# RizaXudayi/VarNet

Measured on AMD Instinct MI355X. Metric: training-points/sec (test-funcs x quad-pts), 2D+t AD-PDE, higher is better.
Workload: dtype f32

## Files before the change

varnet_amd/csrc/vn_fused16.hip:

```cpp
#include "vn_internal.h"
#include "vn_fused16_common.h"

namespace {
using namespace vn16;

constexpr int TSW = 132;
__host__ __device__ constexpr int t_rows(int KS) { return KS == 13 ? 52 : KS <= 8 ? 33 : 64; }
template <int KS>
__device__ __forceinline__ int trow(int pos) {
  if (KS == 13) return pos < 50 ? pos : pos == 52 ? 51 : 50;
  if (KS <= 8) return pos < 32 ? pos : 32;
  return pos;
}
__host__ __device__ constexpr bool fullpos(int KS) { return KS == 16 || KS == 8; }
__host__ __device__ constexpr int vones(int KS) {
  if (fullpos(KS)) return 4 * KS - 1;
  for (int p = 0; p < 64; ++p)
    if (vks(p) >= KS) return p;
  return -1;
}
static_assert(vfeat(63) == 63 && vfeat(31) == 31 && vpos(7, 3) == 31, "position 4*KS-1 is feature 4*KS-1");
#ifndef VN_MERGED_ROUNDS
#define VN_MERGED_ROUNDS 1
#endif
__host__ __device__ constexpr bool merged_rounds(int L, int KS) { return VN_MERGED_ROUNDS && KS <= 8 && L >= 2; }
__host__ __device__ constexpr bool bf_sweeps(int L, int KS) { return KS == 13 && L >= 2 && L <= 5; }

template <int L, int KS>
struct Lay {
  static constexpr int HP = 4 * KS;
  static constexpr bool BF = bf_sweeps(L, KS);
  static constexpr int HPWS = BF ? IMG / 4 : al4(HP * WS);
  static constexpr int W1_OFF = 0;
  static constexpr int WH_OFF = al4(8 * WS);
  static constexpr int BI_OFF = WH_OFF + (L - 1) * HPWS;
  static constexpr int WO_OFF = BI_OFF + L * 64;
  static constexpr int MISC_OFF = WO_OFF + al4(4 * KS);
  static constexpr int T_OFF = MISC_OFF + 256;
  static constexpr int G1_SZ = (4 * KS0 + 1) * HP;
  static constexpr int GH_SZ = (HP + 1) * HP;
  static constexpr int GO_OFF = G1_SZ + (L - 1) * GH_SZ;
  static constexpr int G_SZ = al4(GO_OFF + HP + 1);
  static constexpr bool MERGE = merged_rounds(L, KS);
  static constexpr int T_IMG = (MERGE ? 2 : 1) * 2 * t_rows(KS) * TSW;
  static constexpr int T_H13 = (KS == 13) ? 27 * (NW * 64 + 4) : 0;
  static constexpr int T_MAX = T_IMG > T_H13 ? T_IMG : T_H13;
  static constexpr int T_SZ_SHARED = al4(T_MAX > G_SZ ? T_MAX : G_SZ);
  static constexpr bool G_LOW = (T_OFF + T_SZ_SHARED > 160 * 256) && G_SZ <= MISC_OFF;
  static constexpr int T_SZ = G_LOW ? al4(T_MAX) : T_SZ_SHARED;
  static constexpr int G_OFF = G_LOW ? 0 : T_OFF;
  static constexpr int SLOT_SZ = NW * 2 * 4 * 64;
  static constexpr bool SLOT_IN_T = G_LOW || (T_SZ - al4(G_SZ) >= SLOT_SZ);
  static constexpr int SLOT_OFF = G_LOW ? T_OFF : (SLOT_IN_T ? T_OFF + al4(G_SZ) : 0);
  static_assert(SLOT_IN_T || SLOT_SZ <= MISC_OFF, "thin-layer slots fit neither behind the gradient image nor over the weight images");
  static constexpr int ST_OFF = T_OFF + T_SZ;
  static constexpr int ST_LAYER = NW * 2 * 64 * 4;
  static constexpr int ST_FIT = (160 * 256 - ST_OFF) / ST_LAYER;
  static constexpr int NST = (BF || (KS != 13 && KS != 16) || L < 3) ? 0 : (ST_FIT < L - 1 ? ST_FIT : L - 1);
  static constexpr int TOTAL = ST_OFF + NST * ST_LAYER;
  static constexpr int NSTG = (!BF || L < 3) ? 0 : 1;
  static constexpr int NSTK = BF ? NSTG : NST;
  static_assert(!BF || TOTAL <= 160 * 256, "bf16-piece images must fit the LDS");
};


struct LaneC {
  int g, c;
  int offF;
  int offB0;
  int twr;
};

template <int KSA, int KSB>
struct WG {
  static constexpr int ONES = vones(KSA);
  static constexpr int MTA0 = (mtiles(KSA) > (ONES >> 4) + 1) ? mtiles(KSA) : (ONES >> 4) + 1;
  static constexpr int MTA = MTA0 == 3 ? 4 : MTA0;
  static constexpr int NTB0 = mtiles(KSB);
  static constexpr int NTB = NTB0 == 3 ? 4 : NTB0;
  static constexpr int NT = MTA * NTB;
  static constexpr int TPW = (NT >= NW) ? NT / NW : 1;
  static constexpr int NS = (NT >= NW) ? 1 : NW / NT;
  static constexpr int PTS = TILE / NS;
  static constexpr int PG = PTS / 4;
  static constexpr int ones_m = ONES >> 4;
  static constexpr int ones_i = ONES & 3;
  static constexpr int ones_g = (ONES >> 2) & 3;
  static_assert(NT == 1 || NT == 2 || NT == 4 || NT == 8 || NT == 16, "tile count must divide the waves");
  static_assert(NT < NW || NTB % TPW == 0, "a wave's tiles must share a row tile");
};



template <int KS>
__device__ __forceinline__ void t_write(float* T, const LaneC& lc, int ks, float v) {
  if (KS == 13 && ks == 12) {
    if (lc.g < 2) T[lc.twr + (48 - lc.g) * TSW] = v;
  } else {
    T[lc.twr + vpos(ks, 0) * TSW] = v;
  }
}

template <int KSA, int KSB, bool RAWA, bool TANH, bool MERGE, int NACC, class AV, class BV>
__device__ __forceinline__ void wgrad_layer(const AV& av, const AV& azd, const BV& bv, const BV& bt, float* TA,
                                            float* TB, const LaneC& lc, int wave, f32x4 (&acc)[NACC], bool ones_row) {
  using W = WG<KSA, KSB>;
  static_assert(NACC == W::TPW, "accumulator count");
  const int t0 = (W::NT >= NW) ? wave * W::TPW : wave % W::NT;
  const int sidx = (W::NT >= NW) ? 0 : wave / W::NT;
  const int m = t0 / W::NTB, n0 = t0 % W::NTB;
  const int goff = (W::PG == 32) ? 64 * (lc.g & 1) + 32 * (lc.g >> 1) : lc.g * W::PG;
  const int rdA = trow<KSA>(16 * m + lc.c) * TSW + sidx * W::PTS + goff;
  int rdBt[W::TPW];
#pragma unroll
  for (int t = 0; t < W::TPW; ++t) rdBt[t] = trow<KSB>(16 * (n0 + t) + lc.c) * TSW + sidx * W::PTS + goff;
  constexpr int T2 = MERGE ? 2 * t_rows(KSB) * TSW : 0;
  auto contract = [&](const float* TAh, const float* TBh) {
    f32x4 a4 = *reinterpret_cast<const f32x4a*>(&TAh[rdA]);
    f32x4 b4[W::TPW];
#pragma unroll
    for (int t = 0; t < W::TPW; ++t) b4[t] = *reinterpret_cast<const f32x4a*>(&TBh[rdBt[t]]);
#pragma unroll
    for (int j = 0; j < W::PG / 4; ++j) {
      f32x4 an = a4, bn[W::TPW];
#pragma unroll
      for (int t = 0; t < W::TPW; ++t) bn[t] = b4[t];
      if (j + 1 < W::PG / 4) {
        an = *reinterpret_cast<const f32x4a*>(&TAh[rdA + 4 * (j + 1)]);
#pragma unroll
        for (int t = 0; t < W::TPW; ++t)
          bn[t] = *reinterpret_cast<const f32x4a*>(&TBh[rdBt[t] + 4 * (j + 1)]);
      }
      __builtin_amdgcn_sched_barrier(0);
#pragma unroll
      for (int e = 0; e < 4; ++e)
#pragma unroll
        for (int t = 0; t < W::TPW; ++t) acc[t] = mfma16(a4[e], b4[t][e], acc[t]);
      __builtin_amdgcn_sched_barrier(0);
      a4 = an;
#pragma unroll
      for (int t = 0; t < W::TPW; ++t) b4[t] = bn[t];
    }
  };
#pragma unroll
// ... 372 lines not shown
  float* WH = lds + LY::WH_OFF;
  float* BI = lds + LY::BI_OFF;
  float* WO = lds + LY::WO_OFF;
  float* sInt = lds + LY::MISC_OFF;
  float* TA = lds + LY::T_OFF;
  float* TB = TA + t_rows(KS) * TSW;
  const unsigned t_base_bytes = (unsigned)((LY::T_OFF + wave * 64) * 4);
  float* Gacc = lds + LY::G_OFF;

  const int q = A.integ_num;
  const int pq_l = (wave * CW + (lane & 15)) % q;
  const int tf_l = (wave * CW + (lane & 15)) / q;
  const float tab_dnt = A.time_dependent ? A.fedNt[pq_l] : 0.f;
  const float tab_w = A.feW ? A.feW[pq_l] : 1.f;
  const float tab_N = A.feN[pq_l];
  const float bo = A.theta[net.boff[L + 1]];
  {
    const int d_in = net.d_in, H1 = net.H[1];
    constexpr int NSRC = (LY::HP * LY::HP + NTHREADS - 1) / NTHREADS;
    static_assert(8 * 64 <= NTHREADS, "layer 1: one parameter per thread");
    float v1 = 0.f, vh[L > 1 ? L - 1 : 1][NSRC];
    if (tid < d_in * H1) v1 = A.theta[net.woff[1] + tid];
#pragma unroll
    for (int l = 2; l <= (LY::BF ? 1 : L); ++l) {
      const int n = net.H[l - 1] * net.H[l];
      const float* src = A.theta + net.woff[l];
#pragma unroll
      for (int it = 0; it < NSRC; ++it) {
        const int j = tid + it * NTHREADS;
        vh[l - 2][it] = j < n ? src[j] : 0.f;
      }
    }
    static_assert(L * 64 <= NTHREADS && 4 * KS <= NTHREADS, "one bias / output weight per thread");
    float vb = 0.f, vo = 0.f;
    if (tid < L * 64) {
      const int l = tid / 64 + 1, idx = tid % 64;
      const int mt = idx >> 4, g = (idx >> 2) & 3, r = idx & 3;
      const int ks = 4 * mt + r, f = 4 * ks + g;
      vb = (ks < KS && f < net.H[l]) ? A.theta[net.boff[l] + f] : 0.f;
    }
    if (tid < 4 * KS) vo = (tid < net.H[L]) ? A.theta[net.woff[L + 1] + tid] : 0.f;
    static_assert(LY::BI_OFF % 4 == 0 && LY::T_OFF % 4 == 0 && LY::T_SZ % 4 == 0, "16-byte zero fill");
    const f32x4 z4 = {0.f, 0.f, 0.f, 0.f};
    for (int i = tid; i < (LY::BF ? LY::WH_OFF : LY::BI_OFF) / 4; i += NTHREADS) reinterpret_cast<f32x4a*>(lds)[i] = z4;
    for (int i = tid; i < LY::T_SZ / 4; i += NTHREADS) reinterpret_cast<f32x4a*>(lds + LY::T_OFF)[i] = z4;
    __syncthreads();
    if (tid < d_in * H1) {
      const int k = tid / H1, f = tid - k * H1;
      W1[k * WS + vpos(f >> 2, f & 3)] = v1;
    }
    if constexpr (LY::BF) stage_split_hidden<L, true>(net, A.theta, reinterpret_cast<char*>(WH), tid);
#pragma unroll
    for (int l = 2; l <= (LY::BF ? 1 : L); ++l) {
      float* Wl = WH + (l - 2) * LY::HPWS;
      const int Hout = net.H[l], n = net.H[l - 1] * Hout;
      const int dq = NTHREADS / Hout, dr = NTHREADS - dq * Hout;
      int k = tid / Hout, f = tid - k * Hout;
#pragma unroll
      for (int it = 0; it < NSRC; ++it) {
        if (tid + it * NTHREADS < n) Wl[k * WS + vpos(f >> 2, f & 3)] = vh[l - 2][it];
        f += dr; k += dq;
        if (f >= Hout) { f -= Hout; ++k; }
      }
    }
    if (tid < L * 64) BI[tid] = vb;
    if (tid < 4 * KS) WO[tid] = vo;
  }
  __syncthreads();

  LaneC lc;
  lc.g = lane >> 4;
  lc.c = lane & 15;
  lc.offF = lc.g * WS + lc.c;
  static_assert(16 * GE::MTM <= LY::HP, "backward fragment rows stay inside the weight image");
  static_assert(vfeat(16 + 5) == 16 + vfeat(5), "row tile m holds features fin(c) + 16m");
  lc.offB0 = vfeat(lc.c) * WS + 4 * lc.g;
  lc.twr = 4 * lc.g * TSW + wave * CW + lc.c;

  using W1G = WG<KS0, KS>;
  using WHG = WG<KS, KS>;
  constexpr bool HID13 = (KS == 13);
  constexpr int NHACC = HID13 ? 2 : WHG::TPW;
  constexpr int ST_L = LY::ST_LAYER / 4;
  f32x4a* stash = (LY::BF ? reinterpret_cast<f32x4a*>(A.stash) + (long)blockIdx.x * LY::NSTG * ST_L
                          : reinterpret_cast<f32x4a*>(lds + LY::ST_OFF)) + wave * 2 * 64 + lane;
  constexpr int WIN = 2 * IMG;
  const int rowb = split_row_base(lc.g, lc.c), trb = split_tr_base(lc.g, lc.c);
  auto win_base = [&](int lane_base, int l) {
    const char* wh = reinterpret_cast<const char*>(WH);
    if (l - 2 < 2) return wh + lane_base + (l - 2) * IMG;
    int b = lane_base + WIN;
    asm volatile("" : "+v"(b));
    return wh + b + (l - 4) * IMG;
  };
  f32x4 wacc1[W1G::TPW], wacch[L > 1 ? L - 1 : 1][NHACC];
  float woacc = 0.f, boacc = 0.f;
#pragma unroll
  for (int t = 0; t < W1G::TPW; ++t) wacc1[t] = f32x4{0.f, 0.f, 0.f, 0.f};
#pragma unroll
  for (int l = 0; l < (L > 1 ? L - 1 : 1); ++l)
#pragma unroll
    for (int t = 0; t < NHACC; ++t) {
      wacch[l][t] = f32x4{0.f, 0.f, 0.f, 0.f};
      if (l < LY::NSTK) stash[l * ST_L + t * 64] = wacch[l][t];
    }

  const bool thin_in = net.d_in <= 3;
  bool ones_h[L > 1 ? L - 1 : 1];
#pragma unroll
  for (int l = 2; l <= L; ++l) ones_h[l - 2] = !fullpos(KS) || net.H[l - 1] < 4 * KS;
  float bsum_h[L > 1 ? L - 1 : 1];
#pragma unroll
  for (int l = 0; l < (L > 1 ? L - 1 : 1); ++l) bsum_h[l] = 0.f;
  const int TT = TILE / q;
  const int TPTS = TT * q;
  const bool qtree = (TILE % q) == 0;
  const long ntiles_i = A.mode ? (A.nT + TILE - 1) / TILE : (A.n_k + TT - 1) / TT;
  const long ntiles = ntiles_i + (A.mode == 1 ? 0 : (A.nB + TILE - 1) / TILE);
  float loss_var = 0.f, loss_bc = 0.f, loss_ic = 0.f;
  const long nI = A.nB - A.bDof;
  const float cb = A.bDof > 0 ? 2.f * A.w0 * A.biDimVal / (float)A.bDof : 0.f;
  const float ci = nI > 0 ? 2.f * A.w1 * A.biDimVal / (float)nI : 0.f;
  enum : unsigned {
    FL_MODE1 = 1u << 0, FL_MODE2 = 1u << 1, FL_DIR = 1u << 2, FL_TD = 1u << 3, FL_DNTROW = 1u << 4, FL_SRC = 1u << 5,
    FL_NROW = 1u << 6, FL_QTREE = 1u << 7, FL_DETJV = 1u << 8, FL_LOSSVEC = 1u << 9, FL_SEEDU = 1u << 10, FL_SEEDUD = 1u << 11,
    FL_OUTU = 1u << 12, FL_OUTUD = 1u << 13, FL_THIN_IN = 1u << 14
  };
  const unsigned flags = (A.mode == 1 ? FL_MODE1 : 0u) | (A.mode == 2 ? FL_MODE2 : 0u) | (A.dir >= 0 ? FL_DIR : 0u) |
                         (A.time_dependent ? FL_TD : 0u) | (A.dNtrow ? FL_DNTROW : 0u) | (A.src ? FL_SRC : 0u) |
                         (A.Nrow ? FL_NROW : 0u) | (qtree ? FL_QTREE : 0u) | (A.detJv ? FL_DETJV : 0u) |
                         (A.lossVec ? FL_LOSSVEC : 0u) | (A.seed_u ? FL_SEEDU : 0u) | (A.seed_ud ? FL_SEEDUD : 0u) |
                         (A.out_u ? FL_OUTU : 0u) | (A.out_ud ? FL_OUTUD : 0u) | (thin_in ? FL_THIN_IN : 0u);
  auto fl = [flags](unsigned bits) {
    unsigned f = flags;
    asm volatile("" : "+s"(f));
    return (f & bits) != 0u;
  };
  auto sc = [](int v) {
    asm volatile("" : "+s"(v));
    return v;
  };
  const int d_in_s = net.d_in, dim_s = net.dim, dir_s = A.dir;

  for (long tile = blockIdx.x; tile < ntiles; tile += gridDim.x) {
    asm volatile("" ::: "memory");
    const bool interior = tile < ntiles_i;
    const bool moded = fl(FL_MODE1 | FL_MODE2);
    const long r0 = (interior && !moded) ? tile * TPTS : (interior ? tile : tile - ntiles_i) * TILE;
    const long nrows = interior ? A.nT : A.nB;
    const int pt = wave * CW + lc.c;
    const long row = r0 + pt;
    const bool valid = row < nrows && (!interior || moded || pt < TPTS);

    float xin[KS0], gin[KS0];
    {
      const float* Xp = interior ? A.X : A.Xb;
#pragma unroll
      for (int s = 0; s < KS0; ++s) {
        const int f = 4 * s + lc.g;
        xin[s] = (valid && f < sc(d_in_s)) ? Xp[row * net.d_in + f] : 0.f;
        if (fl(FL_DIR)) gin[s] = (valid && interior && f == sc(dir_s)) ? 1.f : 0.f;
        else gin[s] = (valid && interior && f < sc(dim_s)) ? A.G[row * net.dim + f] : 0.f;
      }
    }

    PA<KS> a[L], zd[L];

    auto layer1_raw = [&](const float (&xi)[KS0], const float (&gi)[KS0], f32x4 (&ov)[GE::MT], f32x4 (&ot)[GE::MT]) {
#pragma unroll
      for (int m = 0; m < GE::MT; ++m) {
        ov[m] = *reinterpret_cast<const f32x4a*>(&BI[m * 16 + lc.g * 4]);
        ot[m] = f32x4{0.f, 0.f, 0.f, 0.f};
      }
#pragma unroll
      for (int s = 0; s < KS0; ++s) {
        if (4 * s < sc(d_in_s)) {
#pragma unroll
          for (int m = 0; m < GE::MT; ++m) {
            const float wf = W1[4 * s * WS + lc.offF + 16 * m];
            ov[m] = mfma16(wf, xi[s], ov[m]);
            ot[m] = mfma16(wf, gi[s], ot[m]);
          }
        }
      }
    };

    f32x4 pv[GE::MT], ptn[GE::MT];
    layer1_raw(xin, gin, pv, ptn);
#pragma unroll
    for (int l = 2; l <= L; ++l) {
      if constexpr (LY::BF) {
        const char* rl = win_base(rowb, l);
        f32x4 nv[GE::MT], nt[GE::MT];
#pragma unroll
        for (int m = 0; m < GE::MT; ++m) {
          nv[m] = *reinterpret_cast<const f32x4a*>(&BI[(l - 1) * 64 + m * 16 + lc.g * 4]);
          nt[m] = f32x4{0.f, 0.f, 0.f, 0.f};
        }
#pragma unroll
        for (int qf = 0; qf < 2; ++qf) {
          u32x4 Bv[3], Bt[3];
#pragma unroll
          for (int e = 0; e < 4; ++e) {
            const int k0 = 8 * qf + 2 * e;
            if (k0 >= KS) {
#pragma unroll
              for (int p = 0; p < 3; ++p) { Bv[p][e] = 0u; Bt[p][e] = 0u; }
              continue;
            }
            const int t = k0 >> 2, i = k0 & 3;
            const bool full = k0 + 1 < KS;
            const float a0 = act_fin<TANH>(act_exp<TANH>(pv[t][i]));
            const float a1 = full ? act_fin<TANH>(act_exp<TANH>(pv[t][i + 1])) : 0.f;
            const float z0 = ptn[t][i], z1 = full ? ptn[t][i + 1] : 0.f;
            a[l - 2].p[k0 >> 1] = f32x2{a0, a1};
            zd[l - 2].p[k0 >> 1] = f32x2{z0, z1};
            u32 h, md, lo;
            split2(a0, a1, h, md, lo);
            Bv[0][e] = h; Bv[1][e] = md; Bv[2][e] = lo;
            split2(act_d1<TANH>(a0) * z0, act_d1<TANH>(a1) * z1, h, md, lo);
            Bt[0][e] = h; Bt[1][e] = md; Bt[2][e] = lo;
          }
#pragma unroll
          for (int mt = 0; mt < GE::MT; ++mt) {
            const u32x4 (*const Bs[2])[3] = {&Bv, &Bt};
            f32x4* const as[2] = {&nv[mt], &nt[mt]};
            if (mt == 3) {
              three_folded<2>(split_frag_row1(rl, 0, qf, mt), Bs, as);
              continue;
            }
            u32x4 Af[3];
            split_frag_row(rl, qf, mt, Af);
            six<2>(Af, Bs, as);
          }
        }
        fold_rows(nv[3]);
        fold_rows(nt[3]);
#pragma unroll
        for (int m = 0; m < GE::MT; ++m) { pv[m] = nv[m]; ptn[m] = nt[m]; }
        continue;
      }
      const float* Wl = WH + (l - 2) * LY::HPWS;
      int k_in = (net.H[l - 1] + 3) >> 2, m_out = (net.H[l] + 15) >> 4;
      f32x4 nv[GE::MT], nt[GE::MT];
#pragma unroll
      for (int m = 0; m < GE::MT; ++m) {
        nv[m] = *reinterpret_cast<const f32x4a*>(&BI[(l - 1) * 64 + m * 16 + lc.g * 4]);
        nt[m] = f32x4{0.f, 0.f, 0.f, 0.f};
      }
      constexpr int NP = PA<KS>::NP;
      auto zin2 = [&](int j) { return f32x2{pv[(2 * j) >> 2][(2 * j) & 3], pv[(2 * j) >> 2][((2 * j) & 3) + 1]}; };
      auto zdin2 = [&](int j) { return f32x2{ptn[(2 * j) >> 2][(2 * j) & 3], ptn[(2 * j) >> 2][((2 * j) & 3) + 1]}; };
      float wf[GE::MTM], we[GE::NVE], ev[GE::NVE], et[GE::NVE];
#pragma unroll
      for (int m = 0; m < GE::MTM; ++m) wf[m] = Wl[lc.offF + 16 * m];
#pragma unroll
      for (int v = 0; v < GE::NVE; ++v) {
        we[v] = GE::EDGE ? Wl[lc.offF - lc.c + GE::EPOS + 4 * v] : 0.f;
        ev[v] = 0.f;
        et[v] = 0.f;
      }
      f32x2 cs2 = act_fin2<TANH>(act_exp2<TANH>(zin2(0)));
      f32x2 cq2 = act_d1_2<TANH>(cs2) * zdin2(0);
      a[l - 2].p[0] = cs2;
      zd[l - 2].p[0] = zdin2(0);
      f32x2 s1 = (NP > 1) ? act_fin2<TANH>(act_exp2<TANH>(zin2(1))) : f32x2{0.f, 0.f};
      f32x2 e2 = (NP > 2) ? act_exp2<TANH>(zin2(2)) : f32x2{0.f, 0.f};
      f32x2 e3 = {0.f, 0.f};
#pragma unroll
      for (int ks = 0; ks < KS; ++ks) {
        const int j = ks >> 1;
        float wn[GE::MTM], wen[GE::NVE];
#pragma unroll
        for (int m = 0; m < GE::MTM; ++m) wn[m] = (ks + 1 < KS) ? Wl[4 * (ks + 1) * WS + lc.offF + 16 * m] : 0.f;
#pragma unroll
        for (int v = 0; v < GE::NVE; ++v)
          wen[v] = (GE::EDGE && ks + 1 < KS) ? Wl[4 * (ks + 1) * WS + lc.offF - lc.c + GE::EPOS + 4 * v] : 0.f;
        const float cs = cs2[ks & 1], cq = cq2[ks & 1];
        __builtin_amdgcn_sched_barrier(0);
        if (GE::live_k(ks, k_in)) {
#pragma unroll
          for (int m = 0; m < GE::MTM; ++m) {
            if (!GE::live_m(m, m_out)) continue;
            nv[m] = mfma16(wf[m], cs, nv[m]);
            nt[m] = mfma16(wf[m], cq, nt[m]);
          }
        }
        if (GE::EDGE) {
#pragma unroll
          for (int v = 0; v < GE::NVE; ++v) { ev[v] += we[v] * cs; et[v] += we[v] * cq; }
        }
        if ((ks & 1) == 0) {
          if (j + 3 < NP) e3 = act_exp2<TANH>(zin2(j + 3));
          __builtin_amdgcn_sched_barrier(0);
        } else {
          f32x2 s2 = s1, q1 = cq2;
          if (j + 2 < NP) s2 = act_fin2<TANH>(e2);
          if (j + 1 < NP) {
            const f32x2 zz = zdin2(j + 1);
            q1 = act_d1_2<TANH>(s1) * zz;
            a[l - 2].p[j + 1] = s1;
            zd[l - 2].p[j + 1] = zz;
          }
          __builtin_amdgcn_sched_barrier(0);
          cs2 = s1; cq2 = q1; s1 = s2; e2 = e3;
        }
#pragma unroll
        for (int m = 0; m < GE::MTM; ++m) wf[m] = wn[m];
#pragma unroll
        for (int v = 0; v < GE::NVE; ++v) we[v] = wen[v];
      }
      if (GE::EDGE) {
        nv[GE::MT - 1][0] += edge_reduce_scatter<GE::NVE>(ev, lc.g);
        nt[GE::MT - 1][0] = edge_reduce_scatter<GE::NVE>(et, lc.g);
      }
// ... 99 lines not shown

    PA<KS> zb, zdb;
#pragma unroll
    for (int j = 0; j < PA<KS>::NP; ++j) {
      const bool full = 2 * j + 1 < KS;
      const f32x2 wv = {WO[4 * (2 * j) + lc.g], full ? WO[4 * (2 * j + 1) + lc.g] : 0.f};
      const f32x2 av = opaque2(a[L - 1].p[j]);
      const f32x2 sp = act_d1_2<TANH>(av);
      const f32x2 ab = wv * f32x2{ubar, ubar}, adb = wv * f32x2{udbar, udbar};
      const f32x2 zq = adb * sp;
      zdb.p[j] = zq;
      zb.p[j] = ab * sp + zq * act_d2r_2<TANH>(av) * zd[L - 1].p[j];
      const f32x2 c2 = av * f32x2{ubar, ubar} + (sp * zd[L - 1].p[j]) * f32x2{udbar, udbar};
      const float s0 = rowsum16(c2[0]);
      woacc += (lc.c == 2 * j) ? s0 : 0.f;
      if (2 * j + 1 < KS) {
        const float s1 = rowsum16(c2[1]);
        woacc += (lc.c == 2 * j + 1) ? s1 : 0.f;
      }
    }
    boacc += rowsum16(ubar);
    if constexpr (HID13) { if (!epi_barrier) __syncthreads(); }
#pragma unroll
    for (int l = L; l >= 2; --l) {
      if (l == 2 && L > 2) {
        float xr[KS0], gr[KS0];
#pragma unroll
        for (int s = 0; s < KS0; ++s) { xr[s] = opaque(xin[s]); gr[s] = opaque(gin[s]); }
        f32x4 rv[GE::MT], rt[GE::MT];
        layer1_raw(xr, gr, rv, rt);
#pragma unroll
        for (int j = 0; j < PA<KS>::NP; ++j) {
          a[0].p[j] = act_fin2<TANH>(act_exp2<TANH>(pairOf(rv, j)));
          zd[0].p[j] = pairOf(rt, j);
        }
      }
      if constexpr (HID13) {
        if (l - 2 < LY::NSTK) {
          f32x4 acc2[2] = {stash[(l - 2) * ST_L], stash[(l - 2) * ST_L + 64]};
          h13_wgrad_layer<TANH, !LY::BF>(a[l - 2], zd[l - 2], zb, zdb, TA, lc, wave, lane, t_base_bytes, acc2);
          stash[(l - 2) * ST_L] = acc2[0];
          stash[(l - 2) * ST_L + 64] = acc2[1];
        } else {
          h13_wgrad_layer<TANH, !LY::BF>(a[l - 2], zd[l - 2], zb, zdb, TA, lc, wave, lane, t_base_bytes, wacch[l - 2]);
        }
      }
      else if constexpr (NHACC == 2) {
        if (l - 2 < LY::NSTK) {
          f32x4 acc2[2] = {stash[(l - 2) * ST_L], stash[(l - 2) * ST_L + 64]};
          wgrad_layer<KS, KS, false, TANH, LY::MERGE>(a[l - 2], zd[l - 2], zb, zdb, TA, TB, lc, wave, acc2, ones_h[l - 2]);
          stash[(l - 2) * ST_L] = acc2[0];
          stash[(l - 2) * ST_L + 64] = acc2[1];
        } else {
          wgrad_layer<KS, KS, false, TANH, LY::MERGE>(a[l - 2], zd[l - 2], zb, zdb, TA, TB, lc, wave, wacch[l - 2], ones_h[l - 2]);
        }
      }
      else wgrad_layer<KS, KS, false, TANH, LY::MERGE>(a[l - 2], zd[l - 2], zb, zdb, TA, TB, lc, wave, wacch[l - 2], ones_h[l - 2]);
      if constexpr (fullpos(KS)) {
        if (!ones_h[l - 2]) thin_bias<KS>(zb, TA, TB, lc, wave, lane, bsum_h[l - 2]);
      }
      f32x4 accv[GE::MT], acct[GE::MT];
#pragma unroll
      for (int m = 0; m < GE::MT; ++m) { accv[m] = f32x4{0.f, 0.f, 0.f, 0.f}; acct[m] = f32x4{0.f, 0.f, 0.f, 0.f}; }
      if constexpr (LY::BF) {
        const char* tl = win_base(trb, l);
#pragma unroll
        for (int qf = 0; qf < 2; ++qf) {
          u32x4 Bz[3], Bzd[3];
#pragma unroll
          for (int e = 0; e < 4; ++e) {
            const int k0 = 8 * qf + 2 * e;
            if (k0 >= KS) {
#pragma unroll
              for (int p = 0; p < 3; ++p) { Bz[p][e] = 0u; Bzd[p][e] = 0u; }
              continue;
            }
            const bool full = k0 + 1 < KS;
            u32 h, md, lo;
            split2(zb[k0], full ? zb[k0 + 1] : 0.f, h, md, lo);
            Bz[0][e] = h; Bz[1][e] = md; Bz[2][e] = lo;
            split2(zdb[k0], full ? zdb[k0 + 1] : 0.f, h, md, lo);
            Bzd[0][e] = h; Bzd[1][e] = md; Bzd[2][e] = lo;
          }
#pragma unroll
          for (int mt = 0; mt < GE::MT; ++mt) {
            const u32x4 (*const Bs[2])[3] = {&Bz, &Bzd};
            f32x4* const as[2] = {&accv[mt], &acct[mt]};
            if (mt == 3) {
              three_folded<2>(split_frag_tr1(tl, 0, qf, mt), Bs, as);
              continue;
            }
            u32x4 At[3];
            split_frag_tr(tl, qf, mt, At);
            six<2>(At, Bs, as);
          }
        }
        fold_rows(accv[3]);
        fold_rows(acct[3]);
      } else {
      const float* Wl = WH + (l - 2) * LY::HPWS;
      int k_out = (net.H[l] + 3) >> 2, m_in = (net.H[l - 1] + 15) >> 4;
      float wf[GE::MTM], we[GE::NVE], ev[GE::NVE], et[GE::NVE];
#pragma unroll
      for (int m = 0; m < GE::MTM; ++m) wf[m] = Wl[lc.offB0 + 16 * m * WS + vpos(0, 0)];
#pragma unroll
      for (int v = 0; v < GE::NVE; ++v) {
        we[v] = GE::EDGE ? Wl[(4 * (KS - 1) + v) * WS + 4 * lc.g + vpos(0, 0)] : 0.f;
        ev[v] = 0.f;
        et[v] = 0.f;
      }
#pragma unroll
      for (int ks = 0; ks < KS; ++ks) {
        float wn[GE::MTM], wen[GE::NVE];
#pragma unroll
        for (int m = 0; m < GE::MTM; ++m) wn[m] = (ks + 1 < KS) ? Wl[lc.offB0 + 16 * m * WS + vpos(ks + 1, 0)] : 0.f;
#pragma unroll
        for (int v = 0; v < GE::NVE; ++v)
          wen[v] = (GE::EDGE && ks + 1 < KS) ? Wl[(4 * (KS - 1) + v) * WS + 4 * lc.g + vpos(ks + 1, 0)] : 0.f;
        __builtin_amdgcn_sched_barrier(0);
        if (GE::live_k(ks, k_out)) {
#pragma unroll
          for (int m = 0; m < GE::MTM; ++m) {
            if (!GE::live_m(m, m_in)) continue;
            accv[m] = mfma16(wf[m], zb[ks], accv[m]);
            acct[m] = mfma16(wf[m], zdb[ks], acct[m]);
          }
        }
        if (GE::EDGE) {
#pragma unroll
          for (int v = 0; v < GE::NVE; ++v) { ev[v] += we[v] * zb[ks]; et[v] += we[v] * zdb[ks]; }
        }
        __builtin_amdgcn_sched_barrier(0);
#pragma unroll
        for (int m = 0; m < GE::MTM; ++m) wf[m] = wn[m];
#pragma unroll
        for (int v = 0; v < GE::NVE; ++v) we[v] = wen[v];
      }
      if (GE::EDGE) {
        accv[GE::MT - 1][0] = edge_reduce_scatter<GE::NVE>(ev, lc.g);
        acct[GE::MT - 1][0] = edge_reduce_scatter<GE::NVE>(et, lc.g);
      }
      }
#pragma unroll
      for (int j = 0; j < PA<KS>::NP; ++j) {
        const int ks = 2 * j;
        if (ks + 1 < KS) {
          const f32x2 av = opaque2(a[l - 2].p[j]);
          const f32x2 sp = act_d1_2<TANH>(av);
          const f32x2 ab = {accv[ks >> 2][ks & 3], accv[ks >> 2][(ks & 3) + 1]};
          const f32x2 adb = {acct[ks >> 2][ks & 3], acct[ks >> 2][(ks & 3) + 1]};
          const f32x2 zq = adb * sp;
          zdb.p[j] = zq;
          zb.p[j] = ab * sp + zq * act_d2r_2<TANH>(av) * zd[l - 2].p[j];
        } else {
          const float av = opaque(a[l - 2][ks]);
          const float sp = act_d1<TANH>(av);
          const float ab = accv[ks >> 2][ks & 3], adb = acct[ks >> 2][ks & 3];
          zdb.set(ks, adb * sp);
          zb.set(ks, ab * sp + adb * sp * act_d2r<TANH>(av) * zd[l - 2][ks]);
        }
      }
    }
    if (fl(FL_THIN_IN)) thin_wgrad_in<KS>(xin, gin, zb, zdb, TA, TB, lc, wave, lane, wacc1[0]);
    else wgrad_layer<KS0, KS, true, TANH, LY::MERGE>(xin, gin, zb, zdb, TA, TB, lc, wave, wacc1, true);
  }

  __syncthreads();
  for (int i = tid; i < (LY::G_LOW ? LY::G_SZ : LY::T_SZ); i += NTHREADS) lds[LY::G_OFF + i] = 0.f;
  __syncthreads();
  float* SL = lds + LY::SLOT_OFF;
#pragma unroll
  for (int i = 0; i < 4; ++i) {
    SL[((wave * 2 + 0) * 4 + i) * 64 + lane] = thin_in ? wacc1[0][i] : 0.f;
    SL[((wave * 2 + 1) * 4 + i) * 64 + lane] = (i == 0) ? woacc : boacc;
  }
  if constexpr (HID13) {
// ... 160 lines not shown
```

varnet_amd/csrc/vn_fused16_common.h:

```cpp
#pragma once
#include "vn_internal.h"

#include <atomic>

typedef float f32x4 __attribute__((ext_vector_type(4)));
typedef f32x4 f32x4a __attribute__((may_alias));

namespace vn16 {

constexpr int NW = 8;
constexpr int NTHREADS = 64 * NW;
constexpr int TILE = 128;
constexpr int CW = 16;
constexpr int WS = 65;
constexpr int KS0 = 2;

__host__ __device__ constexpr int al4(int x) { return (x + 3) & ~3; }
__host__ __device__ constexpr int vpos(int ks, int g) { return 16 * (ks >> 2) + 4 * g + (ks & 3); }
__host__ __device__ constexpr int vks(int pos) { return 4 * (pos >> 4) + (pos & 3); }
__host__ __device__ constexpr int vfeat(int pos) { return 4 * vks(pos) + ((pos >> 2) & 3); }

__host__ __device__ constexpr bool layout_ties_ksteps_and_tiles_to_features() {
  for (int ks = 0; ks < 16; ++ks)
    for (int g = 0; g < 4; ++g)
// ... 74 lines not shown
  __device__ __forceinline__ float operator[](int i) const { return p[i >> 1][i & 1]; }
  __device__ __forceinline__ void set(int i, float v) { p[i >> 1][i & 1] = v; }
};
__device__ __forceinline__ f32x2 opaque2(f32x2 x) {
  asm("" : "+v"(x));
  return x;
}
template <bool TANH>
__device__ __forceinline__ f32x2 act_exp2(f32x2 z) {
  const float c = TANH ? -2.8853900817779268f : -1.4426950408889634f;
  const f32x2 t = z * f32x2{c, c};
  return f32x2{__builtin_amdgcn_exp2f(t[0]), __builtin_amdgcn_exp2f(t[1])};
}
template <bool TANH>
__device__ __forceinline__ f32x2 act_fin2(f32x2 e) {
  const f32x2 d = e + f32x2{1.f, 1.f};
  const f32x2 s = {__builtin_amdgcn_rcpf(d[0]), __builtin_amdgcn_rcpf(d[1])};
  return TANH ? (s * f32x2{2.f, 2.f} - f32x2{1.f, 1.f}) : s;
}
template <bool TANH>
__device__ __forceinline__ f32x2 act_d1_2(f32x2 a) {
  const f32x2 one = {1.f, 1.f};
  return TANH ? (one - a * a) : (a - a * a);
}
template <bool TANH>
__device__ __forceinline__ f32x2 act_d2r_2(f32x2 a) {
  const f32x2 one = {1.f, 1.f}, two = {2.f, 2.f};
  return TANH ? (-two * a) : (one - two * a);
}

__device__ __forceinline__ float rowsum4(float x) {
  float a = x, b = x;
  asm volatile("s_nop 1\n\tv_permlane16_swap_b32 %0, %1" : "+v"(a), "+v"(b));
  const float s = a + b;
  float c = s, d = s;
  asm volatile("s_nop 1\n\tv_permlane32_swap_b32 %0, %1" : "+v"(c), "+v"(d));
  return c + d;
}

template <int CTRL>
__device__ __forceinline__ float dpp_f32(float x) {
  return __builtin_bit_cast(float, __builtin_amdgcn_update_dpp(0, __builtin_bit_cast(int, x), CTRL, 0xf, 0xf, true));
}

__device__ __forceinline__ float rowsum16(float x) {
  x += dpp_f32<0xB1>(x);
  x += dpp_f32<0x4E>(x);
  x += dpp_f32<0x141>(x);
  x += dpp_f32<0x140>(x);
  return x;
}

__device__ __forceinline__ f32x4 mfma16(float a, float b, f32x4 c) {
  return __builtin_amdgcn_mfma_f32_16x16x4f32(a, b, c, 0, 0, 0);
}

template <int NV>
__device__ __forceinline__ float edge_reduce_scatter(const float (&e)[NV], int g) {
  if constexpr (NV == 2) {
    const float keep = (g & 1) ? e[1] : e[0], give = (g & 1) ? e[0] : e[1];
    float t = keep + __shfl_xor(give, 16, 64);
    t += __shfl_xor(t, 32, 64);
    return g < 2 ? t : 0.f;
  } else {
    static_assert(NV == 4, "edge features: 2 or 4");
    const bool odd = (g & 1) != 0;
    const float k0 = odd ? e[1] : e[0], k1 = odd ? e[3] : e[2];
    const float g0 = odd ? e[0] : e[1], g1 = odd ? e[2] : e[3];
    const float a = k0 + __shfl_xor(g0, 16, 64);
    const float b = k1 + __shfl_xor(g1, 16, 64);
    const bool hi = (g & 2) != 0;
    return (hi ? b : a) + __shfl_xor(hi ? a : b, 32, 64);
  }
}

typedef short bf16x8 __attribute__((ext_vector_type(8)));
typedef short s16x4 __attribute__((ext_vector_type(4)));
typedef unsigned u32;
typedef u32 u32x4 __attribute__((ext_vector_type(4)));
typedef u32x4 u32x4a __attribute__((may_alias));

constexpr int BLK = 1024;
constexpr int IMG = 24 * BLK;

__device__ __forceinline__ u32 fu(float x) { return __builtin_bit_cast(u32, x); }
__device__ __forceinline__ float uf(u32 x) { return __builtin_bit_cast(float, x); }
__device__ __forceinline__ u32 pack_hi(u32 u1, u32 u0) { return __builtin_amdgcn_perm(u1, u0, 0x07060302u); }

__device__ __forceinline__ void split2(float x0, float x1, u32& h, u32& m, u32& l) {
  const u32 u0 = fu(x0), u1 = fu(x1);
  h = pack_hi(u1, u0);
  const float r0 = x0 - uf(u0 & 0xffff0000u), r1 = x1 - uf(u1 & 0xffff0000u);
  const u32 v0 = fu(r0), v1 = fu(r1);
  m = pack_hi(v1, v0);
  const float s0 = r0 - uf(v0 & 0xffff0000u), s1 = r1 - uf(v1 & 0xffff0000u);
  l = pack_hi(fu(s1), fu(s0));
}

__device__ __forceinline__ f32x4 mfma_bf16(u32x4 a, u32x4 b, f32x4 c) {
  return __builtin_amdgcn_mfma_f32_16x16x32_bf16(__builtin_bit_cast(bf16x8, a), __builtin_bit_cast(bf16x8, b), c, 0, 0, 0);
}

template <int N>
__device__ __forceinline__ void six(const u32x4 (&A)[3], const u32x4 (*const (&B)[N])[3], f32x4* const (&acc)[N]) {
  constexpr int pa[6] = {1, 2, 0, 1, 0, 0}, pb[6] = {1, 0, 2, 0, 1, 0};
#pragma unroll
  for (int i = 0; i < 6; ++i) {
#pragma unroll
    for (int s = 0; s < N; ++s) *acc[s] = mfma_bf16(A[pa[i]], (*B[s])[pb[i]], *acc[s]);
  }
}

template <int L, bool FOLD13 = false>
__device__ __forceinline__ void stage_split_hidden(const VnNet& net, const float* theta, char* img, int tid) {
  static_assert(NTHREADS == 2 * 4 * 4 * 16, "one entry per thread and layer");
  const int q = tid >> 8, mt = (tid >> 6) & 3, g = (tid >> 4) & 3, c = tid & 15;
  const int pos = 16 * mt + c;
  const int fold_r = (FOLD13 && mt == 3) ? (c & 3) : 0;
  const bool ofold = fold_r == 1 || fold_r == 2;
  const int fo = ofold ? 48 + (c >> 2) : vfeat(pos);
  const int ent = (g * 16 + (c ^ (12 * (g & 1)))) * 16;
#pragma unroll
  for (int l = 2; l <= L; ++l) {
    const int Hin = net.H[l - 1], Hout = net.H[l];
    const float* src = theta + net.woff[l];
    float w[8];
#pragma unroll
    for (int j = 0; j < 8; ++j) {
      const int fi = 4 * (8 * q + j) + g;
      w[j] = (fi < Hin && fo < Hout) ? src[fi * Hout + fo] : 0.f;
    }
    u32x4 ph, pm, pl;
#pragma unroll
    for (int jj = 0; jj < 4; ++jj) {
      u32 h, m, lo;
      split2(w[2 * jj], w[2 * jj + 1], h, m, lo);
      ph[jj] = h; pm[jj] = m; pl[jj] = lo;
    }
    if constexpr (FOLD13) {
      if (ofold) {
        ph = fold_r == 1 ? pm : pl;
        pm = u32x4{0u, 0u, 0u, 0u};
        pl = u32x4{0u, 0u, 0u, 0u};
      } else if (q == 1) {
        ph[2] = (ph[2] & 0xffffu) | (pm[2] << 16);
        ph[3] = (ph[3] & 0xffff0000u) | (pl[2] & 0xffffu);
      }
    }
    char* il = img + (l - 2) * IMG;
    *reinterpret_cast<u32x4a*>(il + ((0 * 2 + q) * 4 + mt) * BLK + ent) = ph;
    *reinterpret_cast<u32x4a*>(il + ((1 * 2 + q) * 4 + mt) * BLK + ent) = pm;
    *reinterpret_cast<u32x4a*>(il + ((2 * 2 + q) * 4 + mt) * BLK + ent) = pl;
  }
}

__device__ __forceinline__ int split_row_base(int g, int c) { return (g * 16 + (c ^ (12 * (g & 1)))) * 16; }
__device__ __forceinline__ int split_tr_base(int g, int c) {
  const int tr_r = c >> 2, tr_p = c & 3;
  return (tr_p * 16 + ((4 * g + tr_r) ^ (12 * (tr_p & 1)))) * 16;
}
__device__ __forceinline__ u32x4 split_frag_row1(const char* rl, int p, int q, int mt) {
  return *reinterpret_cast<const u32x4a*>(rl + ((p * 2 + q) * 4 + mt) * BLK);
}
__device__ __forceinline__ void split_frag_row(const char* rl, int q, int mt, u32x4 (&Af)[3]) {
#pragma unroll
  for (int p = 0; p < 3; ++p) Af[p] = split_frag_row1(rl, p, q, mt);
}
__device__ __forceinline__ u32x4 split_frag_tr1(const char* tl, int p, int q, int mt) {
  const char* b0 = tl + ((p * 2 + (mt >> 1)) * 4 + 2 * q) * BLK + 8 * (mt & 1);
  const s16x4 lo4 = __builtin_amdgcn_ds_read_tr16_b64_v4i16((__attribute__((address_space(3))) s16x4*)(b0));
  const s16x4 hi4 = __builtin_amdgcn_ds_read_tr16_b64_v4i16((__attribute__((address_space(3))) s16x4*)(b0 + BLK));
  const unsigned long long l64 = __builtin_bit_cast(unsigned long long, lo4), h64 = __builtin_bit_cast(unsigned long long, hi4);
  return u32x4{(u32)l64, (u32)(l64 >> 32), (u32)h64, (u32)(h64 >> 32)};
}
__device__ __forceinline__ void split_frag_tr(const char* tl, int q, int mt, u32x4 (&At)[3]) {
#pragma unroll
  for (int p = 0; p < 3; ++p) At[p] = split_frag_tr1(tl, p, q, mt);
}

template <int N>
__device__ __forceinline__ void three_folded(const u32x4& A0, const u32x4 (*const (&B)[N])[3], f32x4* const (&acc)[N]) {
#pragma unroll
  for (int p = 2; p >= 0; --p) {
#pragma unroll
    for (int s = 0; s < N; ++s) *acc[s] = mfma_bf16(A0, (*B[s])[p], *acc[s]);
  }
}
__device__ __forceinline__ void fold_rows(f32x4& t) { t[0] = (t[0] + t[1]) + t[2]; }

template <int L_, int KS_, bool TANH_>
struct Inst {
  static constexpr int L = L_, KS = KS_;
  static constexpr bool TANH = TANH_;
};

#define VN16_VISIT(LL, KK) \
  if (net.L == LL && ks == KK) return net.act == VN_ACT_TANH ? f(Inst<LL, KK, true>{}) : f(Inst<LL, KK, false>{});
#define VN16_DEFINE_VISIT(NAME, CASES)            \
  template <class R, class F>                     \
  R NAME(const VnNet& net, R none, F f) {         \
    const int ks = vn_fused16_ks(net);            \
    CASES(VN16_VISIT)                             \
    return none;                                  \
  }
VN16_DEFINE_VISIT(visit_all, VN16_CASES)
VN16_DEFINE_VISIT(visit_f32_point, VN16_F32_POINT_CASES)
VN16_DEFINE_VISIT(visit_split, VN16_SPLIT_CASES)
#undef VN16_DEFINE_VISIT
#undef VN16_VISIT

template <auto KERNEL, bool OCC = false>
hipError_t allow_lds_once(size_t lds_bytes, int* occ = nullptr) {
  static std::atomic<unsigned long long> attr_done{0};
  static std::atomic<int> occ_cached{1};
  int dev = 0;
  (void)hipGetDevice(&dev);
  const unsigned long long bit = 1ull << (dev & 63);
  if (!(attr_done.load(std::memory_order_acquire) & bit)) {
    hipError_t e = hipFuncSetAttribute((const void*)KERNEL, hipFuncAttributeMaxDynamicSharedMemorySize, (int)lds_bytes);
    if (e != hipSuccess) return e;
    if (OCC) {
      int nb = 1;
      if (hipOccupancyMaxActiveBlocksPerMultiprocessor(&nb, (const void*)KERNEL, NTHREADS, lds_bytes) != hipSuccess) {
        (void)hipGetLastError();
        nb = 1;
      }
      occ_cached.store(nb < 1 ? 1 : nb, std::memory_order_relaxed);
    }
    attr_done.fetch_or(bit, std::memory_order_release);
  }
  if (occ) *occ = occ_cached.load(std::memory_order_relaxed);
  return hipSuccess;
}

template <auto KERNEL, bool OCC, class ARGS>
hipError_t launch_chunks(const ARGS& a, long n, size_t lds_bytes, int ncu, int per_cu, hipStream_t s) {
  int occ = 1;
  const hipError_t e = allow_lds_once<KERNEL, OCC>(lds_bytes, &occ);
  if (e != hipSuccess) return e;
  if (per_cu <= 0) per_cu = occ >= 2 ? 2 : 1;
  const long wgs = ((n + CW - 1) / CW + NW - 1) / NW;
  const long cap = (long)ncu * per_cu;
  const int grid = (int)(wgs < cap ? wgs : cap);
  hipLaunchKernelGGL(KERNEL, dim3(grid), dim3(NTHREADS), lds_bytes, s, a);
  return hipGetLastError();
}

}
```

Baseline: 1.030 billion.

## Compact KS=13 bf16 weight images and use k-half MFMA packing for tail rows

For the KS=13 bf16-split path, the weight images shrink from 24 to 20 blocks by dropping empty mid/lo pieces of the folded row tile. The second k-half of each forward and backward sweep is repacked so the sparse tail work runs as five (or three) MFMAs instead of six. The freed LDS lets the gradient stash stay in LDS rather than global memory when it fits, and the immediate-offset window widens to three layers. The cost is a more intricate fragment layout and packing logic that must keep the split-precision sums exact.

```diff
diff --git a/varnet_amd/csrc/vn_fused16.hip b/varnet_amd/csrc/vn_fused16.hip
--- a/varnet_amd/csrc/vn_fused16.hip
+++ b/varnet_amd/csrc/vn_fused16.hip
@@ -30,7 +30,7 @@
 struct Lay {
   static constexpr int HP = 4 * KS;
   static constexpr bool BF = bf_sweeps(L, KS);
-  static constexpr int HPWS = BF ? IMG / 4 : al4(HP * WS);
+  static constexpr int HPWS = BF ? IMGF / 4 : al4(HP * WS);
   static constexpr int W1_OFF = 0;
   static constexpr int WH_OFF = al4(8 * WS);
   static constexpr int BI_OFF = WH_OFF + (L - 1) * HPWS;
@@ -56,10 +56,12 @@
   static constexpr int ST_OFF = T_OFF + T_SZ;
   static constexpr int ST_LAYER = NW * 2 * 64 * 4;
   static constexpr int ST_FIT = (160 * 256 - ST_OFF) / ST_LAYER;
-  static constexpr int NST = (BF || (KS != 13 && KS != 16) || L < 3) ? 0 : (ST_FIT < L - 1 ? ST_FIT : L - 1);
+  static constexpr int NSTB = (BF && L >= 3) ? 1 : 0;
+  static constexpr int NST = BF ? (ST_FIT >= NSTB ? NSTB : 0)
+                                : (((KS != 13 && KS != 16) || L < 3) ? 0 : (ST_FIT < L - 1 ? ST_FIT : L - 1));
   static constexpr int TOTAL = ST_OFF + NST * ST_LAYER;
-  static constexpr int NSTG = (!BF || L < 3) ? 0 : 1;
-  static constexpr int NSTK = BF ? NSTG : NST;
+  static constexpr int NSTG = BF ? NSTB - NST : 0;
+  static constexpr int NSTK = NST + NSTG;
   static_assert(!BF || TOTAL <= 160 * 256, "bf16-piece images must fit the LDS");
 };
 
@@ -598,16 +600,18 @@
   constexpr bool HID13 = (KS == 13);
   constexpr int NHACC = HID13 ? 2 : WHG::TPW;
   constexpr int ST_L = LY::ST_LAYER / 4;
-  f32x4a* stash = (LY::BF ? reinterpret_cast<f32x4a*>(A.stash) + (long)blockIdx.x * LY::NSTG * ST_L
+  f32x4a* stash = (LY::NSTG ? reinterpret_cast<f32x4a*>(A.stash) + (long)blockIdx.x * LY::NSTG * ST_L
                           : reinterpret_cast<f32x4a*>(lds + LY::ST_OFF)) + wave * 2 * 64 + lane;
-  constexpr int WIN = 2 * IMG;
+  constexpr int WINL = 3;
+  static_assert((WINL - 1) * IMGF + 19 * BLK + 8 + 16 <= 65536, "block offsets of the first window are DS immediates");
+  constexpr int WIN = WINL * IMGF;
   const int rowb = split_row_base(lc.g, lc.c), trb = split_tr_base(lc.g, lc.c);
   auto win_base = [&](int lane_base, int l) {
     const char* wh = reinterpret_cast<const char*>(WH);
-    if (l - 2 < 2) return wh + lane_base + (l - 2) * IMG;
+    if (l - 2 < WINL) return wh + lane_base + (l - 2) * IMGF;
     int b = lane_base + WIN;
     asm volatile("" : "+v"(b));
-    return wh + b + (l - 4) * IMG;
+    return wh + b + (l - 2 - WINL) * IMGF;
   };
   f32x4 wacc1[W1G::TPW], wacch[L > 1 ? L - 1 : 1][NHACC];
   float woacc = 0.f, boacc = 0.f;
@@ -737,16 +741,31 @@
             split2(act_d1<TANH>(a0) * z0, act_d1<TANH>(a1) * z1, h, md, lo);
             Bt[0][e] = h; Bt[1][e] = md; Bt[2][e] = lo;
           }
+          if (qf == 1) {
+            u32x4 Kv[3], Kt[3];
+            khalf_pack(Bv, Kv);
+            khalf_pack(Bt, Kt);
+            const u32x4 (*const Ks[2])[3] = {&Kv, &Kt};
+#pragma unroll
+            for (int mi = 0; mi < GE::MT; ++mi) {
+              const int mt = (mi + 3) & 3;
+              f32x4* const as[2] = {&nv[mt], &nt[mt]};
+              const u32x4 Ad = ffrag_row1(rl, 0, 1, mt);
+              if (mt == 3) three_khalf<2>(lo_lo(Ad), Ad, hi_hi(Ad), Ks, as);
+              else five_khalf<2>(lo_lo(Ad), ffrag_row1(rl, 1, 1, mt), ffrag_row1(rl, 2, 1, mt), Ad, hi_hi(Ad), Ks, as);
+            }
+            continue;
+          }
 #pragma unroll
           for (int mt = 0; mt < GE::MT; ++mt) {
             const u32x4 (*const Bs[2])[3] = {&Bv, &Bt};
             f32x4* const as[2] = {&nv[mt], &nt[mt]};
             if (mt == 3) {
-              three_folded<2>(split_frag_row1(rl, 0, qf, mt), Bs, as);
+              three_folded<2>(ffrag_row1(rl, 0, qf, mt), Bs, as);
               continue;
             }
             u32x4 Af[3];
-            split_frag_row(rl, qf, mt, Af);
+            ffrag_row(rl, qf, mt, Af);
             six<2>(Af, Bs, as);
           }
         }
@@ -1012,16 +1031,34 @@
             split2(zdb[k0], full ? zdb[k0 + 1] : 0.f, h, md, lo);
             Bzd[0][e] = h; Bzd[1][e] = md; Bzd[2][e] = lo;
           }
+          if (qf == 1) {
+            u32x4 Kz[3], Kzd[3];
+            khalf_pack(Bz, Kz);
+            khalf_pack(Bzd, Kzd);
+            const u32x4 (*const Ks[2])[3] = {&Kz, &Kzd};
+#pragma unroll
+            for (int mt = 0; mt < GE::MT; ++mt) {
+              f32x4* const as[2] = {&accv[mt], &acct[mt]};
+              const unsigned long long T0 = ffrag_tr_half(tl, 0, 2, mt), E0 = ffrag_tr_half(tl, 0, 3, mt);
+              if (mt == 3) {
+                three_khalf<2>(halves(T0, T0), halves(T0, E0), halves(E0, E0), Ks, as);
+                continue;
+              }
+              const unsigned long long T1 = ffrag_tr_half(tl, 1, 2, mt), T2 = ffrag_tr_half(tl, 2, 2, mt);
+              five_khalf<2>(halves(T0, T0), halves(T1, T1), halves(T2, 0ull), halves(T0, E0), halves(E0, E0), Ks, as);
+            }
+            continue;
+          }
 #pragma unroll
           for (int mt = 0; mt < GE::MT; ++mt) {
             const u32x4 (*const Bs[2])[3] = {&Bz, &Bzd};
             f32x4* const as[2] = {&accv[mt], &acct[mt]};
             if (mt == 3) {
-              three_folded<2>(split_frag_tr1(tl, 0, qf, mt), Bs, as);
+              three_folded<2>(ffrag_tr1(tl, 0, qf, mt), Bs, as);
               continue;
             }
             u32x4 At[3];
-            split_frag_tr(tl, qf, mt, At);
+            ffrag_tr(tl, qf, mt, At);
             six<2>(At, Bs, as);
           }
         }
diff --git a/varnet_amd/csrc/vn_fused16_common.h b/varnet_amd/csrc/vn_fused16_common.h
--- a/varnet_amd/csrc/vn_fused16_common.h
+++ b/varnet_amd/csrc/vn_fused16_common.h
@@ -180,6 +180,8 @@
 
 constexpr int BLK = 1024;
 constexpr int IMG = 24 * BLK;
+constexpr int IMGF = 20 * BLK;
+__host__ __device__ constexpr int fblk(int p, int q, int mt) { return p == 0 ? q * 4 + mt : 8 + ((p - 1) * 2 + q) * 3 + mt; }
 
 __device__ __forceinline__ u32 fu(float x) { return __builtin_bit_cast(u32, x); }
 __device__ __forceinline__ float uf(u32 x) { return __builtin_bit_cast(float, x); }
@@ -240,10 +242,23 @@
         ph = fold_r == 1 ? pm : pl;
         pm = u32x4{0u, 0u, 0u, 0u};
         pl = u32x4{0u, 0u, 0u, 0u};
-      } else if (q == 1) {
+      } else if (q == 1 && mt != 3) {
         ph[2] = (ph[2] & 0xffffu) | (pm[2] << 16);
         ph[3] = (ph[3] & 0xffff0000u) | (pl[2] & 0xffffu);
+        pm[2] = pm[0];
+        pm[3] = pm[1];
+        pl[2] = 0u;
+        pl[3] = 0u;
       }
+    }
+    if constexpr (FOLD13) {
+      char* il = img + (l - 2) * IMGF;
+      *reinterpret_cast<u32x4a*>(il + fblk(0, q, mt) * BLK + ent) = ph;
+      if (mt != 3) {
+        *reinterpret_cast<u32x4a*>(il + fblk(1, q, mt) * BLK + ent) = pm;
+        *reinterpret_cast<u32x4a*>(il + fblk(2, q, mt) * BLK + ent) = pl;
+      }
+      continue;
     }
     char* il = img + (l - 2) * IMG;
     *reinterpret_cast<u32x4a*>(il + ((0 * 2 + q) * 4 + mt) * BLK + ent) = ph;
@@ -286,6 +301,62 @@
 }
 __device__ __forceinline__ void fold_rows(f32x4& t) { t[0] = (t[0] + t[1]) + t[2]; }
 
+__device__ __forceinline__ u32 dup_lo16(u32 x) { return x | (x << 16); }
+__device__ __forceinline__ void khalf_pack(const u32x4 (&B)[3], u32x4 (&K)[3]) {
+  K[0] = u32x4{B[0][0], B[0][1], B[1][0], B[1][1]};
+  K[1] = u32x4{B[2][0], B[2][1], dup_lo16(B[0][2]), B[0][2]};
+  K[2] = u32x4{dup_lo16(B[1][2]), 0u, B[2][2], 0u};
+}
+template <int N>
+__device__ __forceinline__ void five_khalf(const u32x4& Aa, const u32x4& Ab, const u32x4& Ac, const u32x4& Ad, const u32x4& Ae,
+                                           const u32x4 (*const (&K)[N])[3], f32x4* const (&acc)[N]) {
+#pragma unroll
+  for (int s = 0; s < N; ++s) *acc[s] = mfma_bf16(Ac, (*K[s])[0], *acc[s]);
+#pragma unroll
+  for (int s = 0; s < N; ++s) *acc[s] = mfma_bf16(Ab, (*K[s])[0], *acc[s]);
+#pragma unroll
+  for (int s = 0; s < N; ++s) *acc[s] = mfma_bf16(Ae, (*K[s])[2], *acc[s]);
+#pragma unroll
+  for (int s = 0; s < N; ++s) *acc[s] = mfma_bf16(Ad, (*K[s])[1], *acc[s]);
+#pragma unroll
+  for (int s = 0; s < N; ++s) *acc[s] = mfma_bf16(Aa, (*K[s])[0], *acc[s]);
+}
+template <int N>
+__device__ __forceinline__ void three_khalf(const u32x4& At, const u32x4& Ad, const u32x4& Ae, const u32x4 (*const (&K)[N])[3],
+                                            f32x4* const (&acc)[N]) {
+#pragma unroll
+  for (int s = 0; s < N; ++s) *acc[s] = mfma_bf16(Ae, (*K[s])[2], *acc[s]);
+#pragma unroll
+  for (int s = 0; s < N; ++s) *acc[s] = mfma_bf16(Ad, (*K[s])[1], *acc[s]);
+#pragma unroll
+  for (int s = 0; s < N; ++s) *acc[s] = mfma_bf16(At, (*K[s])[0], *acc[s]);
+}
+__device__ __forceinline__ u32x4 lo_lo(const u32x4& a) { return u32x4{a[0], a[1], a[0], a[1]}; }
+__device__ __forceinline__ u32x4 hi_hi(const u32x4& a) { return u32x4{a[2], a[3], a[2], a[3]}; }
+__device__ __forceinline__ u32x4 halves(unsigned long long lo, unsigned long long hi) {
+  return u32x4{(u32)lo, (u32)(lo >> 32), (u32)hi, (u32)(hi >> 32)};
+}
+
+__device__ __forceinline__ u32x4 ffrag_row1(const char* rl, int p, int q, int mt) {
+  return *reinterpret_cast<const u32x4a*>(rl + fblk(p, q, mt) * BLK);
+}
+__device__ __forceinline__ void ffrag_row(const char* rl, int q, int mt, u32x4 (&Af)[3]) {
+#pragma unroll
+  for (int p = 0; p < 3; ++p) Af[p] = ffrag_row1(rl, p, q, mt);
+}
+__device__ __forceinline__ unsigned long long ffrag_tr_half(const char* tl, int p, int mo, int mt) {
+  const s16x4 v = __builtin_amdgcn_ds_read_tr16_b64_v4i16(
+      (__attribute__((address_space(3))) s16x4*)(tl + fblk(p, mt >> 1, mo) * BLK + 8 * (mt & 1)));
+  return __builtin_bit_cast(unsigned long long, v);
+}
+__device__ __forceinline__ u32x4 ffrag_tr1(const char* tl, int p, int q, int mt) {
+  const unsigned long long l64 = ffrag_tr_half(tl, p, 2 * q, mt), h64 = ffrag_tr_half(tl, p, 2 * q + 1, mt);
+  return u32x4{(u32)l64, (u32)(l64 >> 32), (u32)h64, (u32)(h64 >> 32)};
+}
+__device__ __forceinline__ void ffrag_tr(const char* tl, int q, int mt, u32x4 (&At)[3]) {
+#pragma unroll
+  for (int p = 0; p < 3; ++p) At[p] = ffrag_tr1(tl, p, q, mt);
+}
 template <int L_, int KS_, bool TANH_>
 struct Inst {
   static constexpr int L = L_, KS = KS_;
```

Measured after the change: 1.053 billion (median of 6 runs). +2.2%, better.
